# valeoai/PAFUSE

Hardware: AMD Instinct MI355X
Metric: hypotheses/sec through DDIM loop (H3WB 133-kp, P=20, T=10) (higher is better)
Workload: dtype bf16x3 (every fp32 GEMM operand as the exact sum of three bf16 slices, six bf16 MFMA products per fp32-equivalent product, fp32 accumulate; activations, LayerNorm, softmax, attention and everything in memory fp32; the residual stream stored centred on its row means)

## Files before the change

pafuse_amd/csrc/kernels.hpp:

```cpp
#pragma once
#include <hip/hip_runtime.h>
#include <stdint.h>

#include <utility>

namespace pafuse {

typedef float f32x16 __attribute__((ext_vector_type(16)));
typedef float f32x4 __attribute__((ext_vector_type(4)));

constexpr int BK = 32;
constexpr int LDK = 36;

typedef __bf16 bf16x8 __attribute__((ext_vector_type(8)));
__device__ __forceinline__ bf16x8 to_bf16x8(const f32x4 lo, const f32x4 hi) {
    bf16x8 v;
#pragma unroll
    for (int i = 0; i < 4; ++i) v[i] = (__bf16)lo[i], v[4 + i] = (__bf16)hi[i];
    return v;
}

#ifdef PAFUSE_MFMA_K8
typedef __bf16 bf16x4_t __attribute__((ext_vector_type(4)));
typedef short s16x4_t __attribute__((ext_vector_type(4)));
// ... 1444 lines not shown
        }
    sum += __shfl_xor(sum, 16);
    sum += __shfl_xor(sum, 32);
    const float inv = 1.0f / sum;
#pragma unroll
    for (int kt = 0; kt < KT; ++kt)
#pragma unroll
        for (int reg = 0; reg < 4; ++reg) sc[kt][reg] *= inv;

    f32x4 oc[CT];
#pragma unroll
    for (int ct = 0; ct < CT; ++ct) oc[ct] = f32x4{0.f, 0.f, 0.f, 0.f};
#pragma unroll
    for (int kt = 0; kt < KT; ++kt)
#pragma unroll
        for (int reg = 0; reg < 4; ++reg) {
            const float* vrow = Vb + (kt * 16 + 4 * g + reg) * LDV + l15;
#pragma unroll
            for (int ct = 0; ct < CT; ++ct)
                oc[ct] = __builtin_amdgcn_mfma_f32_16x16x4f32(vrow[ct * 16], sc[kt][reg], oc[ct], 0, 0, 0);
        }
    const int q = qt * 16 + l15;
    if (q < p.L) {
        if (p.o_h) {
            uint8_t* const hrow = p.o_h + (base + q * p.tok_stride) * p.C * 4;
#pragma unroll
            for (int ct = 0; ct < CT; ++ct)
                if (ct * 16 + 4 * g < p.d) {
                    const int c = head * p.d + ct * 16 + 4 * g;
                    hsplit_store4(hrow + (c >> 3) * 32, c & 4, oc[ct]);
                }
            return;
        }
        float* orow = p.o + (base + q * p.tok_stride) * p.C + head * p.d + 4 * g;
#pragma unroll
        for (int ct = 0; ct < CT; ++ct)
            if (ct * 16 + 4 * g < p.d) *reinterpret_cast<f32x4*>(orow + ct * 16) = oc[ct];
    }
}

template <int LP, int DP, int NW>
__global__ void __launch_bounds__(NW * 64) attn_kernel(const AttnParams p) {
    PAFUSE_XQ_GUARD();
    constexpr int QT = LP / 16, KT = LP / 16, CT = DP / 16, SD = DP / 16, ITEMS = NW / QT, LDV = DP + 4;
    constexpr int NTHR = NW * 64, C4 = DP / 4;
    static_assert(NW % QT == 0, "waves must be a multiple of the query tiles");
    extern __shared__ __attribute__((aligned(16))) float smem[];
    float* Ks = smem;
    float* Vs = smem + ITEMS * LP * LDV;
    const int tid = threadIdx.x, lane = tid & 63, wave = tid >> 6;
    const int64_t nitems = p.nseq * p.heads;
    const int C3 = 3 * p.C;

    const int il = wave / QT, qt = wave % QT;
    const int64_t item = (int64_t)blockIdx.x * ITEMS + il;
    const bool mine = item < nitems;
    int64_t seq = 0;
    int head = 0;
    if (mine) attn_item<ITEMS>(item, p.nseq, p.heads, seq, head);
    const int64_t base = (seq / p.group) * p.group_stride + (seq % p.group) * p.seq_stride;
    const int l15 = lane & 15, g = lane >> 4;
    f32x4 qf[SD];
    {
        const int q = qt * 16 + l15;
#pragma unroll
        for (int s = 0; s < SD; ++s) {
            qf[s] = f32x4{0.f, 0.f, 0.f, 0.f};
            if (mine && q < p.L && 16 * s + 4 * g < p.d)
                qf[s] = *reinterpret_cast<const f32x4*>(p.qkv + (base + q * p.tok_stride) * C3 + head * p.d + 16 * s +
                                                        4 * g);
        }
    }
    for (int sl = 0; sl < ITEMS; ++sl) {
        const int64_t it2 = (int64_t)blockIdx.x * ITEMS + sl;
        const bool ok = it2 < nitems;
        int64_t seq2 = 0;
        int head2 = 0;
        if (ok) attn_item<ITEMS>(it2, p.nseq, p.heads, seq2, head2);
        const int64_t base2 = (seq2 / p.group) * p.group_stride + (seq2 % p.group) * p.seq_stride;
        for (int idx = tid; idx < LP * C4; idx += NTHR) {
            const int t = idx / C4, c4 = idx % C4;
            f32x4 kv = {0.f, 0.f, 0.f, 0.f}, vv = {0.f, 0.f, 0.f, 0.f};
            if (ok && t < p.L && c4 * 4 < p.d) {
                const float* src = p.qkv + (base2 + t * p.tok_stride) * C3 + head2 * p.d + c4 * 4;
                kv = *reinterpret_cast<const f32x4*>(src + p.C);
                vv = *reinterpret_cast<const f32x4*>(src + 2 * p.C);
            }
            *reinterpret_cast<f32x4*>(Ks + (sl * LP + t) * LDV + c4 * 4) = kv;
            *reinterpret_cast<f32x4*>(Vs + (sl * LP + t) * LDV + c4 * 4) = vv;
        }
    }
    __syncthreads();
    if (!mine) return;
    const float* Kb = Ks + il * LP * LDV;
    attn_tile<KT, SD, CT, LDV>(
        p, qf, [&](int kt, int s) { return *reinterpret_cast<const f32x4*>(Kb + (kt * 16 + l15) * LDV + 16 * s + 4 * g); },
        Vs + il * LP * LDV, qt, base, head, l15, g);
}

constexpr int attn_wave_min_waves(int LP, int DP, int WPB) {
    const int by_lds = (160 * 1024 / (WPB * LP * (DP + 4) * 4) * WPB + 3) / 4, by_regs = LP == 80 ? 3 : 4;
    return by_lds < by_regs ? by_lds : by_regs;
}
template <int LP, int DP, int WPB>
__global__ void __launch_bounds__(WPB * 64, attn_wave_min_waves(LP, DP, WPB)) attn_wave_kernel(const AttnParams p) {
    PAFUSE_XQ_GUARD();
    constexpr int QT = LP / 16, KT = LP / 16, CT = DP / 16, SD = DP / 16, LDV = DP + 4, C4 = DP / 4, VN = LP * C4 / 64;
    static_assert(LP * C4 % 64 == 0, "V rows are loaded by whole waves");
    extern __shared__ __attribute__((aligned(16))) float smem[];
    const int lane = threadIdx.x & 63, wave = threadIdx.x >> 6, l15 = lane & 15, g = lane >> 4;
    const int64_t item = (int64_t)blockIdx.x * WPB + wave;
    if (item >= p.nseq * p.heads) return;
    int64_t seq;
    int head;
    attn_item<WPB>(item, p.nseq, p.heads, seq, head);
    const int64_t base = (seq / p.group) * p.group_stride + (seq % p.group) * p.seq_stride;
    const int C3 = 3 * p.C;
    const float* const qh = p.qkv + head * p.d;
    float* const Vs = smem + wave * LP * LDV;

    auto frag = [&](int t, int off, f32x4(&f)[SD]) {
        const int tok = t * 16 + l15;
#pragma unroll
        for (int s = 0; s < SD; ++s) {
            f[s] = f32x4{0.f, 0.f, 0.f, 0.f};
            if (tok < p.L && 16 * s + 4 * g < p.d)
                f[s] = *reinterpret_cast<const f32x4*>(qh + (base + tok * p.tok_stride) * C3 + off + 16 * s + 4 * g);
        }
    };
    f32x4 qf[2][SD], kf[KT][SD], vv[VN];
    frag(0, 0, qf[0]);
#pragma unroll
    for (int kt = 0; kt < KT; ++kt) frag(kt, p.C, kf[kt]);
#pragma unroll
    for (int i = 0; i < VN; ++i) {
        const int t = (lane + 64 * i) / C4, c4 = (lane + 64 * i) % C4;
        vv[i] = f32x4{0.f, 0.f, 0.f, 0.f};
        if (t < p.L && c4 * 4 < p.d) vv[i] = *reinterpret_cast<const f32x4*>(qh + (base + t * p.tok_stride) * C3 + 2 * p.C + c4 * 4);
    }
#pragma unroll
    for (int i = 0; i < VN; ++i) {
        const int t = (lane + 64 * i) / C4, c4 = (lane + 64 * i) % C4;
        *reinterpret_cast<f32x4*>(Vs + t * LDV + c4 * 4) = vv[i];
    }
    asm volatile("s_waitcnt lgkmcnt(0)" ::: "memory");
#pragma unroll
    for (int t = 0; t < QT; ++t) {
        if (16 * t >= p.L) break;
        if (t + 1 < QT) frag(t + 1, 0, qf[(t + 1) & 1]);
        attn_tile<KT, SD, CT, LDV>(p, qf[t & 1], [&](int kt, int s) { return kf[kt][s]; }, Vs, t, base, head, l15, g);
    }
}

constexpr int ATTN_LONG_LP = 256;
template <int DP>
__global__ void __launch_bounds__(1024) attn_long_kernel(const AttnParams p) {
    PAFUSE_XQ_GUARD();
    constexpr int LP = ATTN_LONG_LP, T = LP / 16, SD = DP / 16, CT = DP / 16, LDV = DP + 4, C4 = DP / 4;
    extern __shared__ __attribute__((aligned(16))) float smem[];
    float* Ks = smem;
    float* Vs = smem + LP * LDV;
    const int tid = threadIdx.x, lane = tid & 63, w = tid >> 6, l15 = lane & 15, g = lane >> 4;
    int64_t seq;
    int head;
    attn_item<1>((int64_t)blockIdx.x, p.nseq, p.heads, seq, head);
    const int64_t base = (seq / p.group) * p.group_stride + (seq % p.group) * p.seq_stride;
    const int C3 = 3 * p.C, nt = (p.L + 15) / 16;
    f32x4 qf[SD];
    {
        const int q = 16 * w + l15;
#pragma unroll
        for (int s = 0; s < SD; ++s) {
            qf[s] = f32x4{0.f, 0.f, 0.f, 0.f};
            if (q < p.L && 16 * s + 4 * g < p.d)
                qf[s] = *reinterpret_cast<const f32x4*>(p.qkv + (base + (int64_t)q * p.tok_stride) * C3 + head * p.d + 16 * s + 4 * g);
        }
    }
    for (int idx = tid; idx < nt * 16 * C4; idx += 1024) {
        const int t = idx / C4, c4 = idx % C4;
        f32x4 kv = {0.f, 0.f, 0.f, 0.f}, vv = {0.f, 0.f, 0.f, 0.f};
        if (t < p.L && c4 * 4 < p.d) {
            const float* src = p.qkv + (base + (int64_t)t * p.tok_stride) * C3 + head * p.d + c4 * 4;
            kv = *reinterpret_cast<const f32x4*>(src + p.C);
            vv = *reinterpret_cast<const f32x4*>(src + 2 * p.C);
        }
        *reinterpret_cast<f32x4*>(Ks + t * LDV + c4 * 4) = kv;
        *reinterpret_cast<f32x4*>(Vs + t * LDV + c4 * 4) = vv;
    }
    __syncthreads();
    if (w >= nt) return;
    f32x4 sc[T];
#pragma unroll
    for (int kt = 0; kt < T; ++kt) {
        sc[kt] = f32x4{0.f, 0.f, 0.f, 0.f};
        if (kt < nt) {
#pragma unroll
            for (int s = 0; s < SD; ++s) {
                const f32x4 kf = *reinterpret_cast<const f32x4*>(Ks + (kt * 16 + l15) * LDV + 16 * s + 4 * g);
#pragma unroll
                for (int j = 0; j < 4; ++j) sc[kt] = __builtin_amdgcn_mfma_f32_16x16x4f32(kf[j], qf[s][j], sc[kt], 0, 0, 0);
            }
        }
    }
    float mx = -INFINITY;
#pragma unroll
    for (int kt = 0; kt < T; ++kt)
#pragma unroll
        for (int reg = 0; reg < 4; ++reg) {
            const float v = kt * 16 + 4 * g + reg < p.L ? sc[kt][reg] * p.scale : -INFINITY;
            sc[kt][reg] = v;
            mx = fmaxf(mx, v);
        }
    mx = fmaxf(mx, __shfl_xor(mx, 16));
    mx = fmaxf(mx, __shfl_xor(mx, 32));
    float sum = 0.f;
#pragma unroll
    for (int kt = 0; kt < T; ++kt)
#pragma unroll
        for (int reg = 0; reg < 4; ++reg) {
            const float e = __builtin_amdgcn_exp2f((sc[kt][reg] - mx) * 1.44269504088896340736f);
            sc[kt][reg] = e;
            sum += e;
        }
    sum += __shfl_xor(sum, 16);
    sum += __shfl_xor(sum, 32);
    const float inv = 1.0f / sum;
    f32x4 oc[CT];
#pragma unroll
    for (int ct = 0; ct < CT; ++ct) oc[ct] = f32x4{0.f, 0.f, 0.f, 0.f};
#pragma unroll
    for (int kt = 0; kt < T; ++kt)
        if (kt < nt) {
#pragma unroll
            for (int reg = 0; reg < 4; ++reg) {
                const float pr = sc[kt][reg] * inv;
                const float* vrow = Vs + (kt * 16 + 4 * g + reg) * LDV + l15;
#pragma unroll
                for (int ct = 0; ct < CT; ++ct) oc[ct] = __builtin_amdgcn_mfma_f32_16x16x4f32(vrow[ct * 16], pr, oc[ct], 0, 0, 0);
            }
        }
    const int q = 16 * w + l15;
    if (q < p.L) {
        float* orow = p.o + (base + (int64_t)q * p.tok_stride) * p.C + head * p.d + 4 * g;
#pragma unroll
        for (int ct = 0; ct < CT; ++ct)
            if (ct * 16 + 4 * g < p.d) *reinterpret_cast<f32x4*>(orow + ct * 16) = oc[ct];
    }
}

struct FqaParams {
    GemmParams g;
    float* o;
    int64_t nseq;
    int L, C, heads, d, nseq_tile;
    int64_t group, group_stride, seq_stride, tok_stride;
    float scale;
};

template <int LP, int DP>
struct FqaTile {
    static constexpr int NB = 3 * DP / 16, LDV = DP + 4, ROWS = 128 + (LP == 48 ? 4 : 0);
    static constexpr int STAGE_BYTES = Tile16<NB>::STAGE_BYTES, QKV_BYTES = 3 * ROWS * LDV * 4;
    static constexpr int LDS_BYTES = STAGE_BYTES > QKV_BYTES ? STAGE_BYTES : QKV_BYTES;
};

template <int LP, int DP>
__global__ void __launch_bounds__(256, 2) fqa_kernel(const FqaParams fp) {
    PAFUSE_XQ_GUARD();
    using FT = FqaTile<LP, DP>;
    constexpr int NB = FT::NB, LDV = FT::LDV, ROWS = FT::ROWS;
    using T = Tile16<NB>;
    constexpr int A_LD = T::A_LD, W_LD = T::W_LD, NTHR = T::NTHR;
    extern __shared__ __attribute__((aligned(16))) float smem[];
    const GemmParams& p = fp.g;
    uint8_t* const As = reinterpret_cast<uint8_t*>(smem);
    uint8_t* const Ws = As + T::A_BYTES;
    const int tid = threadIdx.x, lane = tid & 63, wave = tid >> 6;
    const int c = lane & 15, qd = lane >> 4;
    const int L = fp.L, NSEQ = fp.nseq_tile;
    const int64_t ntiles = (fp.nseq + NSEQ - 1) / NSEQ;
    const int xcd = blockIdx.x & 7, idx = blockIdx.x >> 3;
    const int64_t tile = (int64_t)(idx / fp.heads) * 8 + xcd;
    const int head = idx % fp.heads;
    if (tile >= ntiles) return;
    const int K = p.K, nk = K / 32;
    const int64_t seq0 = tile * NSEQ;
    const int64_t last_seq = fp.nseq - 1;
    auto token_of = [&](int r) -> int64_t {
        int sl = r / L, t = r - sl * L;
        if (sl >= NSEQ) sl = NSEQ - 1, t = L - 1;
        int64_t sq = seq0 + sl;
        if (sq > last_seq) sq = last_seq;
        return (sq / fp.group) * fp.group_stride + (sq % fp.group) * fp.seq_stride + t * fp.tok_stride;
    };

    const float* a_ptr[A_LD];
    int a_dst[A_LD];
#pragma unroll
    for (int i = 0; i < A_LD; ++i) {
        const int g = 2 * wave + (i >> 1), j = 4 * (i & 1) + qd;
        a_ptr[i] = p.A + token_of(16 * g + c) * K + 4 * j;
        a_dst[i] = g * 2048 + (j & 1) * 1024 + ((j >> 1) * 16 + c) * 16;
    }
    const int n0 = head * 3 * DP;
    const uint8_t* const Wsbase = p.Wsplit + (int64_t)n0 * WSPLIT_ROW_BYTES + tid * 16;
    const int64_t ws_chunk = (int64_t)p.N * WSPLIT_ROW_BYTES;
// ... 3691 lines not shown
```

pafuse_amd/csrc/pafuse_hip.hip:

```cpp
#include "../../include/pafuse_hip.h"

#include <hip/hip_runtime.h>

#include <algorithm>
#include <cmath>
#include <cstdarg>
#include <cstdio>
#include <cstdlib>
#include <cstring>
#include <type_traits>

#include "kernels.hpp"
#include "hgemm.hpp"
#include "xgemm.hpp"
#include "sgemm.hpp"
#include "train_kernels.hpp"

using namespace pafuse;

namespace {

thread_local char g_err[512] = "";

int fail(int code, const char* fmt, ...) {
// ... 382 lines not shown
    p.wlayout = WLAYOUT_PLAIN;
#endif
#ifndef PAFUSE_NO_STRIP
    if (strip2_ok(p)) return strip2_bias(p, s);
#endif
    if (p.mode == MODE_BF16X3 && p.wlayout == WLAYOUT_M16) {
        if (p.N % 128 == 0) return launch_gemm16<8, 3>(p, s);
        if (p.N % 96 == 0) return launch_gemm16<6, 3>(p, s);
        if (p.N % 112 == 0) return launch_gemm16<7, 3>(p, s);
        if (p.N % 64 == 0) return launch_gemm16<4, 4>(p, s);
        return launch_gemm16<2, 4>(p, s);
    }
    if (p.mode == MODE_BF16X3) {
        if (p.N % 128 == 0 && p.M >= 4096) return launch_gemm<4, 1, 4, EPI_BIAS, 1, PAFUSE_FC1_MINW, 0, 2>(p, s);
        if (p.N % 64 == 0) return launch_gemm<4, 1, 2, EPI_BIAS, 1, 4, 0, 2>(p, s);
        if (p.N % 96 == 0) return launch_gemm<4, 1, 3, EPI_BIAS, 1, 1, 1, 2>(p, s);
        return launch_gemm<4, 1, 1, EPI_BIAS, 1, 1, 0, 2>(p, s);
    }
    if (p.mode != MODE_F32) {
        if (p.N % 64 == 0) return launch_gemm<4, 1, 2, EPI_BIAS, 1, 5, 0, 1>(p, s);
        if (p.N % 96 == 0) return launch_gemm<4, 1, 3, EPI_BIAS, 1, 1, 1, 1>(p, s);
        return launch_gemm<4, 1, 1, EPI_BIAS, 1, 1, 0, 1>(p, s);
    }
    if (p.N % 64 == 0) return launch_gemm<4, 1, 2, EPI_BIAS, 1, 5>(p, s);
    if (p.N % 96 == 0) return launch_gemm<4, 1, 3, EPI_BIAS, 1, 1, 1>(p, s);
    return launch_gemm<4, 1, 1, EPI_BIAS, 1>(p, s);
}

template <int EPI>
int gemm_rowln_as(const GemmParams& p0, hipStream_t s) {
    GemmParams p = p0;
    if (p.mode == MODE_BF16X3 && (debug_f32_mask() & 2)) p.mode = MODE_F32;
    if (p.M <= 0) return PAFUSE_OK;
    if (p.K % BK || p.K <= 0) return fail(PAFUSE_E_SHAPE, "rowln: K=%d must be a positive multiple of 32", p.K);
    if (p.mode == MODE_F16X2 || p.mode == MODE_BF16X3_IMAGES) {
        if constexpr (EPI == EPI_ROWLN) return p.mode == MODE_F16X2 ? hgemm_rowln(p, s) : xgemm_rowln(p, s);
        else return fail(PAFUSE_E_ARG, "training has no image-pipeline kernels");
    }
    if constexpr (EPI == EPI_ROWLN_TRAIN) {
        if (p.mode == MODE_BF16X3) {
            switch (p.N) {
                case 384: return launch_gemm_dma<2, 2, 6, EPI, 2, 2, 16>(p, s);
                case 256: return launch_gemm_dma<2, 2, 4, EPI, 2, 2, 16>(p, s);
                case 224: if (p.M >= 4096) return launch_gemm_dma<4, 1, 7, EPI, 2, 2, 16>(p, s); break;
                default: break;
            }
            p.mode = MODE_F32;
        }
    }
    if constexpr (EPI == EPI_ROWLN) {
        if (p.mode == MODE_BF16X3) {
            switch (p.N) {
                case 384: return launch_gemm_dma<2, 2, 6, EPI, 2, 2, 16>(p, s);
                case 256: return launch_gemm_dma<2, 2, 4, EPI, 2, 2, 16>(p, s);
                case 288: return launch_gemm_dma<2, 3, 3, EPI, 2, 2, 16>(p, s);
                case 224:
                    return p.M >= 4096 ? launch_gemm_dma<4, 1, 7, EPI, 2, 2, 16>(p, s) : launch_gemm_dma<2, 1, 7, EPI, 2, 2, 16>(p, s);
                case 128: return launch_gemm<1, 4, 1, EPI, 1, 1, 1, 2>(p, s);
                case 64: return launch_gemm<1, 2, 1, EPI, 1, 1, 1, 2>(p, s);
                default: break;
            }
        } else if (p.mode != MODE_F32) {
            switch (p.N) {
                case 384: return launch_gemm<1, 4, 3, EPI, 1, 1, 1, 1>(p, s);
                case 288: return launch_gemm<1, 3, 3, EPI, 1, 1, 1, 1>(p, s);
                case 256: return launch_gemm<2, 2, 4, EPI, 1, 2, 1, 1>(p, s);
                case 224: return launch_gemm<1, 7, 1, EPI, 1, 1, 1, 1>(p, s);
                case 128: return launch_gemm<1, 4, 1, EPI, 1, 1, 1, 1>(p, s);
                case 64: return launch_gemm<1, 2, 1, EPI, 1, 1, 1, 1>(p, s);
                default: break;
            }
        }
    }
    switch (p.N) {
        case 384: return launch_gemm<1, 4, 3, EPI, 1, 1, 1>(p, s);
        case 288: return launch_gemm<1, 3, 3, EPI, 1, 1, 1>(p, s);
        case 256: return launch_gemm<2, 2, 4, EPI, 1, 2, 1>(p, s);
        case 224: return launch_gemm<1, 7, 1, EPI, 1, 1, 1>(p, s);
        case 128: return launch_gemm<1, 4, 1, EPI, 1, 1, 1>(p, s);
        case 64: return launch_gemm<1, 2, 1, EPI, 1, 1, 1>(p, s);
        default: return fail(PAFUSE_E_SHAPE, "no whole-row kernel for channel width %d (have 64,128,224,256,288,384)", p.N);
    }
}

int gemm_rowln(const GemmParams& p, hipStream_t s) { return gemm_rowln_as<EPI_ROWLN>(p, s); }
int gemm_rowln_train(const GemmParams& p, hipStream_t s) { return gemm_rowln_as<EPI_ROWLN_TRAIN>(p, s); }

bool group_ok_rowln(const GemmParams& p) {
    return p.mode == MODE_BF16X3 && p.Wsplit && (p.N == 384 || p.N == 256 || (p.N == 224 && p.M >= 4096)) && p.K % 16 == 0 && p.K > 0 &&
           !(debug_f32_mask() & 2);
}

template <bool ROWLN>
int gemm_group(const GemmParams* ps, int n, hipStream_t s, bool shared_grids) {
    bool ok = ROWLN && shared_grids && n >= 2 && n <= GROUP_MAX;
    for (int i = 0; i < n && ok; ++i) ok = ps[i].M > 0 && group_ok_rowln(ps[i]);
    if (!ok) {
        for (int i = 0; i < n; ++i) {
            const int rc = ROWLN ? gemm_rowln(ps[i], s) : gemm_bias(ps[i], s);
            if (rc) return rc;
        }
        return PAFUSE_OK;
    }
    int order[GROUP_MAX];
    double cost[GROUP_MAX];
    int64_t tiles[GROUP_MAX];
    for (int i = 0; i < n; ++i) {
        const GemmParams& p = ps[i];
        int bm, bn;
        bm = p.N == 224 ? 128 : 64, bn = p.N;
        tiles[i] = (p.M + bm - 1) / bm * (p.N / bn);
        cost[i] = (double)bm * bn * p.K;
        order[i] = i;
    }
    std::sort(order, order + n, [&](int a, int b) { return cost[a] > cost[b]; });
    GroupedGemmParams g{};
    g.n = n;
    int64_t first = 0;
    for (int k = 0; k < n; ++k) {
        g.p[k] = ps[order[k]];
        g.first[k] = (int)first;
        first += (tiles[order[k]] + 7) / 8 * 8;
        if (first > 0x7fffffff) return fail(PAFUSE_E_ARG, "grouped gemm grid out of range");
    }
    g.first[n] = (int)first;
    for (int k = n + 1; k <= GROUP_MAX; ++k) g.first[k] = (int)first;
    constexpr size_t lds = 2 * DmaTile<2, 2, 6, 16>::STAGE_BYTES;
    static_assert(lds >= 2 * DmaTile<2, 2, 4, 16>::STAGE_BYTES && lds >= 2 * DmaTile<4, 1, 7, 16>::STAGE_BYTES && lds <= 80 * 1024, "LDS");
    return launch<grouped_rowln_kernel<EPI_ROWLN>>("grouped_rowln_kernel", (unsigned)first, 256, lds, s, g);
}

bool width_supported(int C) { return C == 384 || C == 288 || C == 256 || C == 224 || C == 128 || C == 64; }

template <int LP, int DP, int NW>
int launch_attn(const AttnParams& p, hipStream_t s) {
    constexpr int ITEMS = NW / (LP / 16);
    constexpr size_t lds = (size_t)2 * ITEMS * LP * (DP + 4) * sizeof(float);
    const int64_t nitems = p.nseq * p.heads;
    const int64_t grid = (nitems + ITEMS - 1) / ITEMS;
    if (grid > 0x7fffffff) return fail(PAFUSE_E_ARG, "attention grid out of range");
    return launch<attn_kernel<LP, DP, NW>>("attn_kernel", (unsigned)grid, NW * 64, lds, s, p);
}

template <int LP, int DP, int WPB>
int launch_attn_wave(const AttnParams& p, hipStream_t s) {
    constexpr size_t lds = (size_t)WPB * LP * (DP + 4) * sizeof(float);
    static_assert(lds <= 64 * 1024 && (160 * 1024 / lds) * WPB >= 12, "LDS");
    const int64_t nitems = p.nseq * p.heads;
    const int64_t grid = (nitems + WPB - 1) / WPB;
    if (grid > 0x7fffffff) return fail(PAFUSE_E_ARG, "attention grid out of range");
    return launch<attn_wave_kernel<LP, DP, WPB>>("attn_wave_kernel", (unsigned)grid, WPB * 64, lds, s, p);
}

template <int DP>
int launch_attn_long(const AttnParams& p, hipStream_t s) {
    constexpr size_t lds = (size_t)2 * ATTN_LONG_LP * (DP + 4) * sizeof(float);
    static_assert(lds <= 160 * 1024, "LDS");
    const int64_t grid = p.nseq * p.heads;
    if (grid > 0x7fffffff) return fail(PAFUSE_E_ARG, "attention grid out of range");
    return launch<attn_long_kernel<DP>>("attn_long_kernel", (unsigned)grid, 1024, lds, s, p);
}

int attention(const AttnParams& p, hipStream_t s) {
    if (p.nseq <= 0) return PAFUSE_OK;
#ifdef PAFUSE_ABL_NO_ATTENTION
    return PAFUSE_OK;
#endif
    if (p.d % 4 || p.d > 48 || p.L > ATTN_LONG_LP || p.L <= 0)
        return fail(PAFUSE_E_SHAPE, "attention: head dim %d (need %%4, <=48) / length %d (need <=%d)", p.d, p.L, ATTN_LONG_LP);
    if (p.L > 144) {
        if (p.o_h) return fail(PAFUSE_E_SHAPE, "attention: no f16x2 image output for sequences of %d > 144 tokens: use mode 2", p.L);
        return p.d <= 32 ? launch_attn_long<32>(p, s) : launch_attn_long<48>(p, s);
    }
    const int dp = p.d <= 32 ? 32 : 48;
    const int lp = p.L <= 32 ? 32 : (p.L <= 48 ? 48 : (p.L <= 80 ? 80 : 144));
    if (lp == 144)
        return dp == 32 ? launch_attn<144, 32, 9>(p, s) : launch_attn<144, 48, 9>(p, s);
    if (dp == 32) {
        if (lp == 32) return launch_attn<32, 32, 4>(p, s);
        if (lp == 48) return launch_attn_wave<48, 32, 4>(p, s);
        return launch_attn_wave<80, 32, 4>(p, s);
    }
    if (lp == 32) return launch_attn_wave<32, 48, 4>(p, s);
    if (lp == 48) return launch_attn_wave<48, 48, 4>(p, s);
    return launch_attn<80, 48, 5>(p, s);
}

constexpr size_t RANGE_FLAG_BYTES = 256;

struct PartBuffers {
    float *x, *xn, *o, *wide;
    int eb;
    float* temb;
    float* pred;
    float* stats;
};

size_t part_buffer_bytes(int64_t M, int C, int B, int eb = 4) {
    return align_up((size_t)M * C * 4) + 2 * align_up((size_t)M * C * eb) + align_up((size_t)M * 3 * C * 4) + align_up((size_t)B * C * 4) +
           align_up((size_t)M * 3 * 4) + align_up((size_t)M * 2 * 4);
}

char* carve_part(char* base, int64_t M, int C, int B, PartBuffers& pb, int eb = 4) {
    pb.eb = eb;
    pb.x = (float*)base;
    base += align_up((size_t)M * C * 4);
    pb.xn = (float*)base;
    base += align_up((size_t)M * C * eb);
    pb.o = (float*)base;
    base += align_up((size_t)M * C * eb);
    pb.wide = (float*)base;
    base += align_up((size_t)M * 3 * C * 4);
    pb.temb = (float*)base;
    base += align_up((size_t)B * C * 4);
    pb.pred = (float*)base;
    base += align_up((size_t)M * 3 * 4);
    pb.stats = (float*)base;
    base += align_up((size_t)M * 2 * 4);
    return base;
}

PartBuffers offset_rows(const PartBuffers& pb, int64_t row0, int C) {
    PartBuffers o = pb;
    const int64_t img = row0 * C * pb.eb / 4;
    o.x = pb.x + row0 * C, o.xn = pb.xn + img, o.o = pb.o + img, o.wide = pb.wide + row0 * 3 * C;
    o.pred = pb.pred + row0 * 3;
    o.stats = pb.stats + row0 * 2;
    return o;
}

static bool ln_folded(const pafuse_mixste2_weights* w) { return w->ste[0].qkv_lt != nullptr; }
static bool h_residual_only(const pafuse_mixste2_weights* w) { return mode_images(w->operand_bf16) && ln_folded(w) && !w->keep_f32_residual; }

static void embed_outputs(EmbedParams& e, int mode, bool folded, bool h_only, float* x, float* xn, void* image, float* stats,
                          int64_t row0, int64_t nrows) {
    e.x = h_only ? nullptr : x, e.xn = xn;
    e.stats = folded ? stats : nullptr;
    e.xh = mode_images(mode) ? reinterpret_cast<uint8_t*>(image) : nullptr;
    e.x_image = mode == MODE_BF16X3_IMAGES;
    e.centre_x = mode == MODE_BF16X3 && folded;
    e.row0 = row0, e.nrows = nrows;
}

int check_weights(const pafuse_mixste2_weights* w, bool training = false) {
    if (!w) return fail(PAFUSE_E_ARG, "null weights");
    static_assert(EMBED_NV * 128 >= 384, "embed kernel covers the widest part");
    if (w->in_chans != 5) return fail(PAFUSE_E_SHAPE, "in_chans must be 5, got %d", w->in_chans);
    if (w->depth < 1 || w->depth > PAFUSE_MAX_DEPTH) return fail(PAFUSE_E_SHAPE, "depth %d out of range", w->depth);
    if (!width_supported(w->channels)) return fail(PAFUSE_E_SHAPE, "channel width %d has no kernel", w->channels);
    if (w->heads <= 0 || w->channels % w->heads) return fail(PAFUSE_E_SHAPE, "heads %d !| C %d", w->heads, w->channels);
    const int d = w->channels / w->heads;
    if (d % 4 || d > 48) return fail(PAFUSE_E_SHAPE, "head dim %d unsupported", d);
    if (w->joints < 1 || w->joints > 144 || w->frames < 1 || w->frames > ATTN_LONG_LP)
        return fail(PAFUSE_E_SHAPE, "sequence lengths J=%d F=%d: J must be in 1..144, F in 1..%d", w->joints, w->frames, ATTN_LONG_LP);
    if (w->operand_bf16 == MODE_F16X2 && w->frames > 144)
        return fail(PAFUSE_E_SHAPE, "f16x2: no attention form for clips of %d > 144 frames: use mode 2", w->frames);
    if (!mode_valid(w->operand_bf16)) return fail(PAFUSE_E_ARG, "matrix-product mode %d", w->operand_bf16);
    if (mode_images(w->operand_bf16)) {
        const int hidden = w->mlp_hidden > 0 ? w->mlp_hidden : 2 * w->channels;
        if (!hgemm_width(w->channels) || !hgemm_plain_n(3 * w->channels) || !hgemm_plain_n(hidden) || hidden % 32)
            return fail(PAFUSE_E_SHAPE, "the image pipelines (f16x2, bf16x3 on images) serve the widths 224 / 256 / 384 with an MLP hidden "
                                        "width that is a multiple of 128 or 224 (got C = %d, hidden = %d): use mode 2", w->channels, hidden);
    }
    if (w->operand_bf16 == MODE_BF16X3_IMAGES && !training) {
        for (int i = 0; i < w->depth; ++i)
            for (const pafuse_block_weights* b : {&w->ste[i], &w->tte[i]})
                if (!b->qkv_hs || !b->qkv_hb) return fail(PAFUSE_E_ARG, "bf16x3 on images needs the head-major qkv image of every block (qkv_hs, qkv_hb)");
        if (!xfqa_has(w->joints, d, w->heads) || !xfqa_has(w->frames, d, w->heads))
            return fail(PAFUSE_E_SHAPE, "bf16x3 on images: no fused qkv + attention form for sequences of %d / %d tokens at head dim %d, %d heads: "
                                        "use mode 2", w->joints, w->frames, d, w->heads);
    }
    if (w->mlp_hidden < 0 || (w->mlp_hidden > 0 && (w->mlp_hidden % 32 || w->mlp_hidden > 3 * w->channels)))
        return fail(PAFUSE_E_SHAPE, "mlp hidden width %d must be a multiple of 32 and at most 3C = %d", w->mlp_hidden, 3 * w->channels);
    if (!(w->qk_scale >= 0.f)) return fail(PAFUSE_E_ARG, "qk_scale must be positive (0 = head_dim^-0.5)");
    if (training && (w->operand_bf16 == MODE_BF16 || mode_images(w->operand_bf16)))
        return fail(PAFUSE_E_ARG, "training runs fp32 ('f32') or split-precision ('bf16x3') products");
    if (mode_split(w->operand_bf16) && !training)
        for (int i = 0; i < w->depth; ++i)
            for (const pafuse_block_weights* b : {&w->ste[i], &w->tte[i]})
                if ((!b->qkv_ws && w->operand_bf16 != MODE_BF16X3_IMAGES) || !b->proj_ws || !b->fc1_ws || !b->fc2_ws)
                    return fail(PAFUSE_E_ARG, "split-precision mode needs the pre-split image of every linear weight "
                                              "(pafuse_split_weights)");
    const bool fold = ln_folded(w);
    for (int i = 0; i < w->depth; ++i)
        for (const pafuse_block_weights* b : {&w->ste[i], &w->tte[i]}) {
            const int set = (b->qkv_lt != nullptr) + (b->fc1_lt != nullptr);
            if (set != (fold ? 2 : 0)) return fail(PAFUSE_E_ARG, "folded-LayerNorm vectors (qkv_lt, fc1_lt) must be set in every block or in none");
        }
    if (fold && !mode_split(w->operand_bf16)) return fail(PAFUSE_E_ARG, "the folded LayerNorm exists in the split-precision modes only");
    return PAFUSE_OK;
}

struct BlockTail {
    const float *post_w, *post_b;
    float post_eps;
    const float* pos;
    int posJ, posF;
    const float *next_w, *next_b;
    float next_eps;
    const float *head_w, *head_b;
    float* out_head;
};

struct BlockLaunch {
    GemmParams qkv, proj, fc1, fc2;
    AttnParams attn;
    FqaParams fqa;
    bool fused;
    MlpParams mlp;
    bool mlp_fused;
};

BlockLaunch make_block(const pafuse_block_weights& bw, const PartBuffers& pb, int64_t M, int C, int heads, int64_t nseq, int L,
                       int64_t group, int64_t group_stride, int64_t seq_stride, int64_t tok_stride, const BlockTail& tail,
                       int mode, int hidden = 0, float qk_scale = 0.f, bool fold = false, bool keep_f32_residual = false) {
    if (hidden <= 0) hidden = 2 * C;
    BlockLaunch b{};
    float* const stats = pb.stats;
    const bool hp = mode_images(mode);
    uint8_t* const xn_h = reinterpret_cast<uint8_t*>(pb.xn);
    const bool h_residual = hp && fold && !keep_f32_residual;
    GemmParams& g = b.qkv;
    g.A = pb.xn, g.W = bw.qkv_w, g.bias = bw.qkv_b, g.out = pb.wide, g.M = M, g.N = 3 * C, g.K = C, g.act = 0;
    g.mode = mode, g.Wsplit = (const uint8_t*)bw.qkv_ws, g.wlayout = WLAYOUT_M16;
    if (fold) g.A = pb.x, g.ln_in = stats, g.bias = bw.qkv_lt;
    if (hp) g.Ah = xn_h, g.Wh = (const uint8_t*)bw.qkv_ws;
    if (fold) g.ln_s = nullptr;
    AttnParams& a = b.attn;
    a.qkv = pb.wide, a.o = pb.o, a.nseq = nseq, a.L = L, a.C = C, a.heads = heads, a.d = C / heads;
    a.group = group, a.group_stride = group_stride, a.seq_stride = seq_stride, a.tok_stride = tok_stride;
    a.scale = qk_scale != 0.f ? qk_scale : 1.0f / sqrtf((float)(C / heads));
    if (hp) a.o_h = reinterpret_cast<uint8_t*>(pb.o);
    b.fused = false;
    if (mode_split(mode) && bw.qkv_hs && bw.qkv_hb && (mode == MODE_BF16X3_IMAGES ? xfqa_has(L, C / heads, heads) : fqa_has(L, C / heads, mode))) {
        const int lp = fqa_lp(L, mode), dp = fqa_dp(C / heads);
        FqaParams& f = b.fqa;
        f.g = g;
        f.g.Wsplit = (const uint8_t*)bw.qkv_hs, f.g.bias = bw.qkv_hb, f.g.ln_s = nullptr;
// ... 2195 lines not shown
```

Before: 108.2.

## Add two-wave per-head attention kernel for 80-token, 48-dim case

Adds attn_pair_kernel, which runs one (sequence, head) item per 128-thread block. The two waves split the query tiles and share a V tile in LDS, while each wave holds all K fragments in registers. The 80-token, 48-dim attention path now uses this kernel in place of the 5-wave attn_kernel. The 32-dim variants sit behind a compile flag. The aim is to raise occupancy and cut per-item LDS and sync overhead, at the cost of heavy register pressure from K fragments and fewer waves per item.

```diff
diff --git a/pafuse_amd/csrc/kernels.hpp b/pafuse_amd/csrc/kernels.hpp
--- a/pafuse_amd/csrc/kernels.hpp
+++ b/pafuse_amd/csrc/kernels.hpp
@@ -1620,6 +1620,53 @@
     }
 }
 
+template <int LP, int DP>
+__global__ void __launch_bounds__(128, LP == 80 && DP == 48 ? 3 : 4) attn_pair_kernel(const AttnParams p) {
+    PAFUSE_XQ_GUARD();
+    constexpr int QT = LP / 16, KT = LP / 16, CT = DP / 16, SD = DP / 16, LDV = DP + 4, C4 = DP / 4, VN = (LP * C4 + 127) / 128;
+    extern __shared__ __attribute__((aligned(16))) float smem[];
+    const int lane = threadIdx.x & 63, wave = __builtin_amdgcn_readfirstlane(threadIdx.x >> 6), l15 = lane & 15, g = lane >> 4;
+    int64_t seq;
+    int head;
+    attn_item<1>((int64_t)blockIdx.x, p.nseq, p.heads, seq, head);
+    const int64_t base = (seq / p.group) * p.group_stride + (seq % p.group) * p.seq_stride;
+    const int C3 = 3 * p.C;
+    const float* const qh = p.qkv + head * p.d;
+
+    auto frag = [&](int t, int off, f32x4(&f)[SD]) {
+        const int tok = t * 16 + l15;
+#pragma unroll
+        for (int s = 0; s < SD; ++s) {
+            f[s] = f32x4{0.f, 0.f, 0.f, 0.f};
+            if (tok < p.L && 16 * s + 4 * g < p.d)
+                f[s] = *reinterpret_cast<const f32x4*>(qh + (base + tok * p.tok_stride) * C3 + off + 16 * s + 4 * g);
+        }
+    };
+    f32x4 qf[2][SD], kf[KT][SD], vv[VN];
+    frag(wave, 0, qf[0]);
+#pragma unroll
+    for (int kt = 0; kt < KT; ++kt) frag(kt, p.C, kf[kt]);
+#pragma unroll
+    for (int i = 0; i < VN; ++i) {
+        const int idx = (int)threadIdx.x + 128 * i, t = idx / C4, c4 = idx % C4;
+        vv[i] = f32x4{0.f, 0.f, 0.f, 0.f};
+        if (t < p.L && c4 * 4 < p.d) vv[i] = *reinterpret_cast<const f32x4*>(qh + (base + t * p.tok_stride) * C3 + 2 * p.C + c4 * 4);
+    }
+#pragma unroll
+    for (int i = 0; i < VN; ++i) {
+        const int idx = (int)threadIdx.x + 128 * i, t = idx / C4, c4 = idx % C4;
+        if (LP * C4 % 128 == 0 || idx < LP * C4) *reinterpret_cast<f32x4*>(smem + t * LDV + c4 * 4) = vv[i];
+    }
+    __syncthreads();
+#pragma unroll
+    for (int i = 0; i < (QT + 1) / 2; ++i) {
+        const int t = 2 * i + wave;
+        if (16 * t >= p.L) break;
+        frag(t + 2, 0, qf[(i + 1) & 1]);
+        attn_tile<KT, SD, CT, LDV>(p, qf[i & 1], [&](int kt, int s) { return kf[kt][s]; }, smem, t, base, head, l15, g);
+    }
+}
+
 constexpr int ATTN_LONG_LP = 256;
 template <int DP>
 __global__ void __launch_bounds__(1024) attn_long_kernel(const AttnParams p) {
diff --git a/pafuse_amd/csrc/pafuse_hip.hip b/pafuse_amd/csrc/pafuse_hip.hip
--- a/pafuse_amd/csrc/pafuse_hip.hip
+++ b/pafuse_amd/csrc/pafuse_hip.hip
@@ -558,6 +558,15 @@
     return launch<attn_wave_kernel<LP, DP, WPB>>("attn_wave_kernel", (unsigned)grid, WPB * 64, lds, s, p);
 }
 
+template <int LP, int DP>
+int launch_attn_pair(const AttnParams& p, hipStream_t s) {
+    constexpr size_t lds = (size_t)LP * (DP + 4) * sizeof(float);
+    static_assert(160 * 1024 / lds >= 8, "LDS");
+    const int64_t grid = p.nseq * p.heads;
+    if (grid > 0x7fffffff) return fail(PAFUSE_E_ARG, "attention grid out of range");
+    return launch<attn_pair_kernel<LP, DP>>("attn_pair_kernel", (unsigned)grid, 128, lds, s, p);
+}
+
 template <int DP>
 int launch_attn_long(const AttnParams& p, hipStream_t s) {
     constexpr size_t lds = (size_t)2 * ATTN_LONG_LP * (DP + 4) * sizeof(float);
@@ -584,12 +593,15 @@
         return dp == 32 ? launch_attn<144, 32, 9>(p, s) : launch_attn<144, 48, 9>(p, s);
     if (dp == 32) {
         if (lp == 32) return launch_attn<32, 32, 4>(p, s);
+#ifdef PAFUSE_ATTN_PAIR_CANDIDATES
+        return lp == 48 ? launch_attn_pair<48, 32>(p, s) : launch_attn_pair<80, 32>(p, s);
+#endif
         if (lp == 48) return launch_attn_wave<48, 32, 4>(p, s);
         return launch_attn_wave<80, 32, 4>(p, s);
     }
     if (lp == 32) return launch_attn_wave<32, 48, 4>(p, s);
     if (lp == 48) return launch_attn_wave<48, 48, 4>(p, s);
-    return launch_attn<80, 48, 5>(p, s);
+    return launch_attn_pair<80, 48>(p, s);
 }
 
 constexpr size_t RANGE_FLAG_BYTES = 256;
```

Result: no change. 107.9 (-0.2%).
